# jina-ai/annlite

Measured on AMD Instinct MI355X. Metric: queries/sec, higher is better.
Workload: dtype f32; 1 GPU; 10000000 x 128-dim float32, PQ m=16 ks=256, euclidean, batch 1024, k=10, exhaustive ADC scan + exact top-k; rows_total=10000000, rows_per_gpu=10000000, batch=1024, k=10, parallelism=row-shard x1, codes_layout=skewed, n_ranks=1, streams=1, query_batches=4, prewarm_steps=64, seed_exchange=False, seed_peers_emulated=0

## Files before the change

### annlite_amd/csrc/scan_q8.hip

```cpp
#include "scan_lists.h"

#ifndef ANNLITE_Q8_EXP
#define ANNLITE_Q8_EXP 0
#endif

namespace annlite {

#ifndef ANNLITE_Q8_WDEPTH
#define ANNLITE_Q8_WDEPTH 16
#endif
#ifndef ANNLITE_Q8_STAGE_DEPTH
#define ANNLITE_Q8_STAGE_DEPTH 8
#endif
#ifndef ANNLITE_Q8_THW_MASK
#define ANNLITE_Q8_THW_MASK 1
#endif
#ifndef ANNLITE_Q8_ROWQ
#define ANNLITE_Q8_ROWQ 1
#endif
#ifndef ANNLITE_Q8_BUILD_UNROLL
#define ANNLITE_Q8_BUILD_UNROLL 2
#endif
#ifndef ANNLITE_Q8_DEPTH
#define ANNLITE_Q8_DEPTH 8
#endif
#ifndef ANNLITE_Q8_SPLIT_DEPTH
#define ANNLITE_Q8_SPLIT_DEPTH 4
#endif
#ifndef ANNLITE_Q8_SPLIT_H
#define ANNLITE_Q8_SPLIT_H 11
#endif
#ifndef ANNLITE_Q8_SPLIT_BIAS
#define ANNLITE_Q8_SPLIT_BIAS 1
#endif

#define ANNLITE_LDS __attribute__((address_space(3)))
template <class T>
__device__ __forceinline__ T ldsv(uint32_t ad) {
    return *(volatile ANNLITE_LDS T *)(uintptr_t)ad;
}
template <class T>
__device__ __forceinline__ void ldsv_st(uint32_t ad, T v) {
    *(volatile ANNLITE_LDS T *)(uintptr_t)ad = v;
}
__device__ __forceinline__ uint32_t lds_add_u32(uint32_t ad, uint32_t v) {
    return __hip_atomic_fetch_add((ANNLITE_LDS uint32_t *)(uintptr_t)ad, v, __ATOMIC_RELAXED, __HIP_MEMORY_SCOPE_WORKGROUP);
}
__device__ __forceinline__ uint32_t lds_base_addr() {
    return (uint32_t)(uintptr_t)(ANNLITE_LDS unsigned char *)g_smem;
}

typedef const ScanArgs __attribute__((address_space(4))) *q8_kernarg_ptr;
__device__ __forceinline__ q8_kernarg_ptr q8_kernarg() { return (q8_kernarg_ptr)__builtin_amdgcn_kernarg_segment_ptr(); }
struct Q8Build {
    const float *lut, *qlom, *qstep, *smax;
    const double *qlo;
    const unsigned long long *gkey;
    int32_t Ks, B, k, target;
    const unsigned long long *gseed0;
    const uint8_t *btab;
};

template <int M, int NW, int NQ>
__device__ __forceinline__ void q8_copy_table(const Q8Build &a, int tile, uint32_t tab_ad, int tid) {
    constexpr int NT = NW * 64;
    static_assert(M == 16 && NQ == 2, "the prebuilt image is the M = 16 kernel's (q8_entry16)");
    constexpr int n16 = kQ8Image16 / 16;
    const int n_g4 = ((a.B + 15) / 16) * 4;
    const u32x4 *src = (const u32x4 *)(a.btab + (int64_t)tile * (int64_t)kQ8Image16);
#pragma unroll 4
    for (int i = tid; i < n16; i += NT) {
        u32x4 v = src[i];
        const int half = i >= 4096 ? 1 : 0;
        const int g4 = tile * (4 * NQ) + (((i & 15) - half) & 1) * 4;
        if (g4 + 3 >= n_g4) {
            if (g4 + 0 >= n_g4) v.x = 0u;
            if (g4 + 1 >= n_g4) v.y = 0u;
            if (g4 + 2 >= n_g4) v.z = 0u;
            v.w = 0u;
        }
        *(ANNLITE_LDS u32x4 *)(uintptr_t)(tab_ad + 16u * (uint32_t)i) = v;
    }
}

template <int M, int NW, int NQ>
__device__ __forceinline__ void q8_build_table(const Q8Build &a, int tile, uint32_t tab_ad, uint32_t inv_ad, uint32_t clip_ad,
                                               int tid) {
    constexpr int RB = M * 16, NT = NW * 64, KHS = NT / M;
    static_assert(NT % M == 0 && KHS % NQ == 0, "build mapping");
    const int m = tid % M, kh0 = tid / M, h = kh0 % NQ;
    const int n_g4 = ((a.B + 15) / 16) * 4;
    float lo_r[16], inv_r[16], clip_r[16];
    const float *src[4];
#pragma unroll
    for (int i = 0; i < 4; ++i) {
        const int g4 = tile * (4 * NQ) + h * 4 + i;
        const bool ok = g4 < n_g4;
        src[i] = a.lut + ((int64_t)(ok ? g4 : 0) * a.Ks * M + m) * 4;
#pragma unroll
        for (int e = 0; e < 4; ++e) {
            lo_r[4 * i + e] = ok ? a.qlom[(int64_t)(g4 * 4 + e) * M + m] : 0.f;
            inv_r[4 * i + e] = ok ? ldsv<float>(inv_ad + 4u * (uint32_t)(h * 16 + 4 * i + e)) : 0.f;
            clip_r[4 * i + e] = ldsv<float>(clip_ad + 4u * (uint32_t)(h * 16 + 4 * i + e));
        }
    }
#pragma unroll ANNLITE_Q8_BUILD_UNROLL
    for (int kh = kh0; kh < a.Ks * NQ; kh += KHS) {
        const int k = kh / NQ;
        uint32_t w[4];
#pragma unroll
        for (int i = 0; i < 4; ++i) {
            const f32x4 v = *(const f32x4 *)(src[i] + (int64_t)k * M * 4);
            uint32_t pk = 0;
#pragma unroll
            for (int e = 0; e < 4; ++e) {
                float t = __builtin_fmaf(v[e] - lo_r[4 * i + e], inv_r[4 * i + e], -0.5f);
                t = __builtin_fminf(t, clip_r[4 * i + e]);
                pk = __builtin_amdgcn_cvt_pk_u8_f32(t, e, pk);
            }
            w[i] = pk;
        }
        uint32_t ad;
        if constexpr (Q8Cfg<M>::M32)
            ad = tab_ad + ((uint32_t)(m >> 4) << 16) + ((uint32_t)k << 8) + (uint32_t)(m & 15) * 16u;
        else if constexpr (M == 16 && NQ == 2) ad = tab_ad + q8_entry16((uint32_t)k, (uint32_t)m, (uint32_t)h);
        else ad = tab_ad + (uint32_t)((k * NQ + h) * RB + m * 16);
        *(ANNLITE_LDS u32x4 *)(uintptr_t)ad = (u32x4){w[0], w[1], w[2], w[3]};
    }
}

template <int NW>
__device__ __forceinline__ void q8_gather_table(const uint8_t *bq, int Ks, uint32_t tab_ad, uint32_t qmap_ad, int tid) {
    const int lane = tid & 63, wave = tid >> 6;
    const uint32_t w = (uint32_t)lane & 3u, g = ((uint32_t)lane >> 2) & 1u, u = ((uint32_t)lane >> 3) & 1u, c2 = (uint32_t)lane >> 4;
    int32_t qb[16];
#pragma unroll
    for (int j = 0; j < 16; ++j) {
        const int b = ldsv<int32_t>(qmap_ad + 4u * (g * 16u + (uint32_t)j));
        qb[j] = b < 0 ? -1 : b * (Ks * 16);
    }
    for (int kk = (int)(2u * c2 + u) + 8 * wave; kk < Ks; kk += 8 * NW) {
        uint32_t r[16];
#pragma unroll
        for (int j = 0; j < 16; ++j)
            r[j] = qb[j] < 0 ? 0u : *(const uint32_t *)(bq + (int64_t)qb[j] + (int64_t)(kk * 16) + (int64_t)(4u * w));
        u32x4 e[4];
#pragma unroll
        for (int v = 0; v < 4; ++v) {
            const uint32_t a = __builtin_amdgcn_perm(r[4 * v + 1], r[4 * v + 0], 0x05010400u);
            const uint32_t a2 = __builtin_amdgcn_perm(r[4 * v + 1], r[4 * v + 0], 0x07030602u);
            const uint32_t c = __builtin_amdgcn_perm(r[4 * v + 3], r[4 * v + 2], 0x05010400u);
            const uint32_t cc2 = __builtin_amdgcn_perm(r[4 * v + 3], r[4 * v + 2], 0x07030602u);
            e[0][v] = __builtin_amdgcn_perm(c, a, 0x05040100u);
            e[1][v] = __builtin_amdgcn_perm(c, a, 0x07060302u);
            e[2][v] = __builtin_amdgcn_perm(cc2, a2, 0x05040100u);
            e[3][v] = __builtin_amdgcn_perm(cc2, a2, 0x07060302u);
        }
#pragma unroll
        for (int t = 0; t < 4; ++t) {
            const uint32_t tt = (uint32_t)t ^ (2u * u);
            const u32x4 val = tt == 0u ? e[0] : tt == 1u ? e[1] : tt == 2u ? e[2] : e[3];
            *(ANNLITE_LDS u32x4 *)(uintptr_t)(tab_ad + q8_entry16((uint32_t)kk, 4u * w + tt, g)) = val;
        }
    }
}

template <int NW>
__device__ __forceinline__ void q8_build_table_wide(const Q8Build &a, int tile, uint32_t tab_ad, uint32_t inv_ad, uint32_t clip_ad,
                                                    int tid) {
    constexpr int M = 64, NT = NW * 64, KPT = NT / M;
    const int m = tid % M, kr = tid / M;
    const int n_g4 = ((a.B + 15) / 16) * 4;
    const uint32_t half_b = (uint32_t)(a.Ks + 1) * 256u;
    float lo_r[8], inv_r[8], clip_r[8];
    const float *src[2];
#pragma unroll
    for (int i = 0; i < 2; ++i) {
        const int g4 = tile * 2 + i;
        const bool ok = g4 < n_g4;
        src[i] = a.lut + ((int64_t)(ok ? g4 : 0) * a.Ks * M + m) * 4;
#pragma unroll
        for (int e = 0; e < 4; ++e) {
            lo_r[4 * i + e] = ok ? a.qlom[(int64_t)(g4 * 4 + e) * M + m] : 0.f;
            inv_r[4 * i + e] = ok ? ldsv<float>(inv_ad + 4u * (uint32_t)(4 * i + e)) : 0.f;
            clip_r[4 * i + e] = ldsv<float>(clip_ad + 4u * (uint32_t)(4 * i + e));
        }
// ... 1057 lines not shown
                    if (arrived == want) break;
                    if ((++idle & 15) == 8) {
                        import_bounds();
                        poll_guard();
                    }
                    __builtin_amdgcn_s_sleep(4);
                }
                q8_publish_global<QT, LK, TL>(fc, lds, lane, pend_o, pend_j);
                epoch_sync(final);
                if (final) break;
                if (ldsv<uint32_t>(lds.ctl)) {
                    if (has_ring && RE == 8u) {
                        const uint32_t tail_v = ldsv<uint32_t>(lds.tails() + 4u * (uint32_t)my_ring);
                        for (uint32_t i = (uint32_t)my_i; i < ((tail_v - head_v) & 0xffffu); i += 4u) {
                            const uint32_t ad = lds.ring + 8u * ((uint32_t)my_ring * kWaveRing + ((head_v + i) & (kWaveRing - 1)));
                            ldsv_st<unsigned long long>(ad, ldsv<unsigned long long>(ad) & ~(0xffffull << 40));
                        }
                    }
                }
                ++epoch;
                epoch_step = a.q8_epoch_mul * epoch_step + (a.q8_epoch_mul - 1);
            }
            if (a.guard && lane == 0) ldsv_st<uint32_t>(lds.seen, ldsv<uint32_t>(lds.seen) + n_seen);
            if (a.dbg && lane == 0 && !(a.dbg_skip & 8)) {
                atomicAdd(a.dbg + 2, (unsigned long long)n_kept);
                atomicAdd(a.dbg + 3, (unsigned long long)n_offered);
                atomicAdd(a.dbg + 4, t_busy);
                atomicAdd(a.dbg + 6, (unsigned long long)n_batches);
            }
        } else {
            constexpr int NF = WIDE ? 4 : 4 * NQ;
            int lane_pin = lane;
            asm volatile("" : "+v"(lane_pin));
            const int s = lane_pin % (WIDE ? 32 : M);
            const int rot_bytes = CB * s;
            const uint32_t bsh = (uint32_t)(rot_bytes & 3);
            bool abit[8];
#pragma unroll
            for (int i = 0; i < 8; ++i) abit[i] = (((rot_bytes >> 2) >> i) & 1) != 0;
            const unsigned long long rmask0 = __ballot(abit[0]), rmask1 = __ballot(abit[1]);
            typedef const ANNLITE_LDS u32x4 *lds_entry_ptr;
            typedef const ANNLITE_LDS u32x2 *lds_entry8_ptr;
            const uint32_t lds0 = lds.tab;
            constexpr bool P16 = M == 16 && NQ == 2 && CB == 1;
            uint32_t mbase[(WIDE || M8 || M32) ? 1 : M];
            if constexpr (!WIDE && !M8 && !M32) {
#pragma unroll
                for (int t = 0; t < M; ++t) mbase[t] = P16 ? q8_entry16(0u, (uint32_t)((s + t) % M), 0u) : lds0 + (uint32_t)(((s + t) % M) * EB);
                if constexpr (P16) {
                    if (lds0 != 0u) __builtin_trap();
                }
            }
            const uint32_t f16 = (M8 && NQ == 2) ? ((uint32_t)lane_pin >> 4) & 1u : 0u;
            uint32_t kx[2] = {0u, 0u}, ky[2] = {0u, 0u};
            if constexpr (M8) {
#pragma unroll
                for (int t = 0; t < 8; ++t) {
                    const uint32_t col = (uint32_t)(((s + t) % 8) * 16) + f16 * 128u;
                    kx[t / 4] |= col << (8 * (t % 4));
                    ky[t / 4] |= (col ^ 128u) << (8 * (t % 4));
                }
                if ((NQ == 2 && lds0 != 0u) || a.Ks > (C16 ? 1024 / NQ : 256)) __builtin_trap();
            }
            uint32_t mcol[(M8 && NQ == 1) ? M : 1];
            if constexpr (M8 && NQ == 1) {
#pragma unroll
                for (int t = 0; t < M; ++t) mcol[t] = lds0 + (uint32_t)(((s + t) % M) * EB);
            }
            uint32_t k32[M32 ? 16 : 1];
            if constexpr (M32) {
#pragma unroll
                for (int j = 0; j < 16; ++j) {
                    const uint32_t s0 = (uint32_t)((s + 2 * j) % 32), s1 = (uint32_t)((s + 2 * j + 1) % 32);
                    k32[j] = ((s0 & 15u) << 4) | ((s0 >> 4) << 8) | ((s1 & 15u) << 20) | ((s1 >> 4) << 24);
                }
                if (lds0 != 0u || a.Ks > 256) __builtin_trap();
            }
            const uint32_t lane_k = 0x00010000u | (uint32_t)((lane_pin & 31) * 8);
            if constexpr (WIDE) {
                if (lds0 != 0u || a.Ks != 256) __builtin_trap();
            }
            const uint32_t *codes32 = (const uint32_t *)a.codes;
            unsigned long long codes_v = (unsigned long long)(uintptr_t)a.codes, valid_v = (unsigned long long)(uintptr_t)a.valid;
            if constexpr (WIDE) asm volatile("" : "+v"(codes_v), "+v"(valid_v));
            const uint32_t n_rows = (uint32_t)a.N;
            const uint32_t n_blocks = item_blocks;
            const bool ilv = a.q8_ilv_log > 0;
            const uint32_t blk_log = ilv ? (uint32_t)a.q8_ilv_log : 26u, blk_msk = (1u << blk_log) - 1u;
            const uint32_t blk_per = ilv ? (uint32_t)a.n_slices << blk_log : 0u;
            const uint32_t blk_off = ilv ? ((uint32_t)slice << blk_log) << 6 : (uint32_t)slice_begin;
            const uint32_t s_end = ilv ? n_rows : (uint32_t)slice_end;
            auto blk_row = [&](uint32_t b) -> uint32_t { return blk_off + (((b >> blk_log) * blk_per + (b & blk_msk)) << 6); };
            auto draw = [&]() -> uint32_t {
                uint32_t v = 0;
                if (lane == 0) v = lds_add_u32(lds.blk_ctr(), 1u);
                return v;
            };
            uint32_t ccur[CW], cnext[CW];
            uint32_t addr[(WIDE || M8 || M32) ? 1 : M];
            auto load_row = [&](uint32_t row, uint32_t (&c)[CW]) {
                if constexpr (ANNLITE_Q8_EXP == 3) {
#pragma unroll
                    for (int i = 0; i < CW; ++i) c[i] = row * 0x9E3779B1u + (uint32_t)i * 0x85EBCA77u;
                    return;
                }
                if (row >= n_rows) row = n_rows - 1;
                typedef const uint32_t __attribute__((address_space(1))) *gptr_t;
                const gptr_t p = (WIDE ? (gptr_t)codes_v : (gptr_t)(uintptr_t)codes32) + (int64_t)row * CW;
                if constexpr (CW == 2) {
                    const u32x2 v = *(const u32x2 __attribute__((address_space(1))) *)p;
                    c[0] = v.x;
                    c[1] = v.y;
                } else {
#pragma unroll
                    for (int i = 0; i < CW / 4; ++i) {
                        const u32x4 v = *(const u32x4 __attribute__((address_space(1))) *)(p + 4 * i);
                        c[4 * i + 0] = v.x;
                        c[4 * i + 1] = v.y;
                        c[4 * i + 2] = v.z;
                        c[4 * i + 3] = v.w;
                    }
                }
            };
            auto make_addr = [&](const uint32_t (&cc)[CW]) {
                if constexpr (P16)
                    static_for<0, M>([&](auto T) {
                        constexpr int t = decltype(T)::value;
                        addr[t] = __builtin_amdgcn_perm(cc[t / 4], mbase[t], 0x0c020000u | ((4u + (uint32_t)(t % 4)) << 8));
                    });
                else if constexpr (!WIDE && !M8 && !M32)
                    static_for<0, CW>([&](auto W) {
                        constexpr int w = decltype(W)::value;
                        uint32_t o0, o1, o2, o3;
                        byte_shl4(cc[w], (uint32_t)ilog2_c(KSTRIDE), o0, o1, o2, o3);
                        addr[4 * w + 0] = mbase[4 * w + 0] + o0;
                        addr[4 * w + 1] = mbase[4 * w + 1] + o1;
                        addr[4 * w + 2] = mbase[4 * w + 2] + o2;
                        addr[4 * w + 3] = mbase[4 * w + 3] + o3;
                    });
            };
            auto load_thw = [&](uint32_t (&t)[NF]) {
                if constexpr (WIDE) {
                    const u32x4 v = *(volatile ANNLITE_LDS u32x4 *)(uintptr_t)lds.shq;
                    t[0] = v.x, t[1] = v.y, t[2] = v.z, t[3] = v.w;
                } else {
#pragma unroll
                    for (int h = 0; h < NQ; ++h) {
                        const u32x4 v = *(volatile ANNLITE_LDS u32x4 *)(uintptr_t)(lds.shq + 16u * ((uint32_t)h ^ f16));
                        t[4 * h + 0] = v.x, t[4 * h + 1] = v.y, t[4 * h + 2] = v.z, t[4 * h + 3] = v.w;
                    }
                }
            };
            constexpr bool BIAS = HS > 0 && ANNLITE_Q8_SPLIT_BIAS != 0;
            auto load_stepw = [&](uint32_t (&t)[NF]) {
                if constexpr (BIAS) {
#pragma unroll
                    for (int h = 0; h < 2; ++h) {
                        const u32x4 v = *(volatile ANNLITE_LDS u32x4 *)(uintptr_t)(lds.qmap + 16u * (uint32_t)h);
                        t[4 * h + 0] = v.x, t[4 * h + 1] = v.y, t[4 * h + 2] = v.z, t[4 * h + 3] = v.w;
                    }
                } else load_thw(t);
            };
            uint32_t thw[NF];
            load_stepw(thw);
            auto row_sums = [&](const uint32_t (&cc)[CW], uint32_t (&sums)[NF]) {
                if constexpr (WIDE) {
                    sums[0] = sums[1] = sums[2] = sums[3] = 0u;
                    constexpr int WDEPTH = ANNLITE_Q8_WDEPTH;
                    static_assert(WDEPTH % 2 == 0 && WDEPTH >= 2 && WDEPTH <= 64, "pairs");
                    u32x2 v[WDEPTH];
                    auto fetch = [&](u32x2 &dst, auto T) {
                        constexpr int t = decltype(T)::value;
                        constexpr int half = t / 32;
                        constexpr uint32_t sel = 0x0c000000u | ((half ? 0x02u : 0x0cu) << 16) | ((4u + (uint32_t)(t % 4)) << 8);
                        const uint32_t ad = __builtin_amdgcn_perm(cc[t / 4], lane_k, sel);
                        dst = *(lds_entry8_ptr)(uintptr_t)(ad + (uint32_t)((t % 32) * 8 + half * 0x100));
                    };
                    static_for<0, WDEPTH>([&](auto I) { fetch(v[decltype(I)::value], I); });
                    u32x2 bs = {0u, 0u};
                    static_for<0, 32>([&](auto P) {
                        constexpr int i = 2 * decltype(P)::value;
                        asm volatile("" ::: "memory");
                        if constexpr (i % 16 == 0) bs = v[i % WDEPTH] + v[(i + 1) % WDEPTH];
                        else bs += v[i % WDEPTH] + v[(i + 1) % WDEPTH];
                        if constexpr (i + WDEPTH < 64) {
                            fetch(v[i % WDEPTH], std::integral_constant<int, i + WDEPTH>{});
                            fetch(v[(i + 1) % WDEPTH], std::integral_constant<int, i + WDEPTH + 1>{});
                        }
                        if constexpr (i % 16 == 14) {
                            sums[0] += bs.x & 0x00ff00ffu;
                            sums[1] += __builtin_amdgcn_perm(0u, bs.x, 0x0c030c01u);
                            sums[2] += bs.y & 0x00ff00ffu;
                            sums[3] += __builtin_amdgcn_perm(0u, bs.y, 0x0c030c01u);
                        }
                    });
                } else if constexpr (M8) {
                    constexpr int DEPTH = ANNLITE_Q8_DEPTH, TOT = NQ * M;
                    u32x4 acc[NQ];
                    u32x4 v[DEPTH];
                    auto fetch = [&](u32x4 &dst, auto I) {
                        constexpr int i = decltype(I)::value, t = i % M, g = i / M;
                        constexpr uint32_t sel = C16 ? 0x0c000000u | ((uint32_t)(4 + 2 * (t % 2) + 1) << 16) | ((uint32_t)(4 + 2 * (t % 2)) << 8) | (uint32_t)(t % 4)
                                                     : 0x0c0c0000u | ((uint32_t)(4 + t % 4) << 8) | (uint32_t)(t % 4);
                        uint32_t ad;
                        if constexpr (NQ == 2) ad = __builtin_amdgcn_perm(cc[C16 ? t / 2 : t / 4], g ? ky[t / 4] : kx[t / 4], sel);
                        else ad = (((t % 2) ? cc[t / 2] >> 16 : cc[t / 2] & 0xffffu) << 7) + mcol[t];
                        dst = *(lds_entry_ptr)(uintptr_t)ad;
                    };
                    static_for<0, DEPTH>([&](auto I) { fetch(v[decltype(I)::value], I); });
                    static_for<0, TOT>([&](auto I) {
                        constexpr int i = decltype(I)::value;
                        asm volatile("" ::: "memory");
                        if constexpr (i % M == 0) acc[i / M] = v[i % DEPTH];
                        else acc[i / M] += v[i % DEPTH];
                        if constexpr (i + DEPTH < TOT) fetch(v[i % DEPTH], std::integral_constant<int, i + DEPTH>{});
                    });
#pragma unroll
                    for (int h = 0; h < NQ; ++h) sums[4 * h + 0] = acc[h].x, sums[4 * h + 1] = acc[h].y, sums[4 * h + 2] = acc[h].z, sums[4 * h + 3] = acc[h].w;
                } else if constexpr (M32) {
                    constexpr int DEPTH = ANNLITE_Q8_DEPTH;
                    u32x4 acc;
                    u32x4 v[DEPTH];
                    auto fetch = [&](u32x4 &dst, auto I) {
                        constexpr int t = decltype(I)::value, b = t % 2;
                        constexpr uint32_t sel = 0x0c000000u | ((uint32_t)(2 * b + 1) << 16) | ((uint32_t)(4 + t % 4) << 8) | (uint32_t)(2 * b);
                        const uint32_t ad = __builtin_amdgcn_perm(cc[t / 4], k32[t / 2], sel);
                        dst = *(lds_entry_ptr)(uintptr_t)ad;
                    };
                    static_for<0, DEPTH>([&](auto I) { fetch(v[decltype(I)::value], I); });
                    static_for<0, M>([&](auto I) {
                        constexpr int i = decltype(I)::value;
                        asm volatile("" ::: "memory");
                        if constexpr (i == 0) acc = v[0];
                        else acc += v[i % DEPTH];
                        if constexpr (i + DEPTH < M) fetch(v[i % DEPTH], std::integral_constant<int, i + DEPTH>{});
                    });
                    sums[0] = acc.x, sums[1] = acc.y, sums[2] = acc.z, sums[3] = acc.w;
                } else {
                    constexpr int DEPTH = ANNLITE_Q8_DEPTH, TOT = NQ * M;
                    constexpr int GOFF = P16 ? 16 : RB;
                    u32x4 acc[NQ];
                    u32x4 v[DEPTH];
                    auto fetch = [&](u32x4 &dst, uint32_t ad) {
                        if constexpr (ANNLITE_Q8_EXP == 2) asm volatile("" : "=v"(dst) : "v"(ad));
                        else dst = *(lds_entry_ptr)(uintptr_t)ad;
                    };
                    static_for<0, DEPTH>([&](auto I) {
                        constexpr int i = decltype(I)::value;
                        fetch(v[i], addr[i % M] + (uint32_t)((i / M) * GOFF));
                    });
                    static_for<0, TOT>([&](auto I) {
                        constexpr int i = decltype(I)::value;
                        asm volatile("" ::: "memory");
                        if constexpr (ANNLITE_Q8_EXP == 1) {
                            asm volatile("" ::"v"(v[i % DEPTH]));
                            if constexpr (i % M == 0) acc[i / M] = (u32x4){thw[4 * (i / M)], thw[4 * (i / M) + 1], thw[4 * (i / M) + 2], thw[4 * (i / M) + 3]};
                        } else {
                            if constexpr (i % M == 0) acc[i / M] = v[i % DEPTH];
                            else acc[i / M] += v[i % DEPTH];
                        }
                        if constexpr (i + DEPTH < TOT) {
                            constexpr int j = i + DEPTH;
                            fetch(v[i % DEPTH], addr[j % M] + (uint32_t)((j / M) * GOFF));
                        }
                    });
#pragma unroll
                    for (int h = 0; h < NQ; ++h) sums[4 * h + 0] = acc[h].x, sums[4 * h + 1] = acc[h].y, sums[4 * h + 2] = acc[h].z, sums[4 * h + 3] = acc[h].w;
                }
            };
            auto hits = [&](uint32_t th, uint32_t sm) -> uint32_t {
                if constexpr (WIDE) return (th - sm) & 0x80008000u;
                else return (th - (sm & 0x7f7f7f7fu)) & ~sm & 0x80808080u;
            };
            auto split_sums = [&](const uint32_t (&cc)[CW], auto T0c, auto T1c, auto DEPTHc, auto ONFLY, uint32_t sp, u32x4 (&acc)[2]) {
                constexpr int T0 = decltype(T0c)::value, TOT = 2 * (decltype(T1c)::value - T0);
                constexpr int DEPTH = decltype(DEPTHc)::value < TOT ? decltype(DEPTHc)::value : TOT;
                if constexpr (P16) {
                    if constexpr (decltype(ONFLY)::value) asm volatile("" : "+v"(sp));
                    u32x4 v[DEPTH];
                    uint32_t ad = 0;
                    auto fetch = [&](u32x4 &dst, auto I) {
                        constexpr int i = decltype(I)::value, t = T0 + i / 2;
                        if constexpr (i % 2 == 0) {
                            uint32_t mb;
                            if constexpr (decltype(ONFLY)::value) {
                                const uint32_t m = (sp + (uint32_t)t) & 15u;
                                mb = ((m & 1u) << 16) | (m << 4);
                            } else mb = mbase[t];
                            ad = __builtin_amdgcn_perm(cc[t / 4], mb, 0x0c020000u | ((4u + (uint32_t)(t % 4)) << 8));
                        }
                        dst = *(lds_entry_ptr)(uintptr_t)(ad + (uint32_t)((i % 2) * 16));
                    };
                    static_for<0, DEPTH>([&](auto I) { fetch(v[decltype(I)::value], I); });
                    static_for<0, TOT>([&](auto I) {
                        constexpr int i = decltype(I)::value;
                        asm volatile("" ::: "memory");
                        if constexpr (T0 == 0 && i < 2) acc[i] = v[i % DEPTH];
                        else acc[i % 2] += v[i % DEPTH];
                        if constexpr (decltype(ONFLY)::value) asm volatile("" : "+v"(acc[i % 2]));
                        if constexpr (i + DEPTH < TOT) fetch(v[i % DEPTH], std::integral_constant<int, i + DEPTH>{});
                    });
                }
            };
            auto split_pass = [&](const u32x4 (&acc)[2]) -> bool {
                uint32_t anyv = 0;
#pragma unroll
                for (int h = 0; h < 2; ++h)
#pragma unroll
                    for (int e = 0; e < 4; ++e) anyv |= (thw[4 * h + e] - (acc[h][e] & 0x7f7f7f7fu)) & ~acc[h][e];
                return (anyv & 0x80808080u) != 0u;
            };
            auto split_pass1 = [&](const u32x4 (&acc)[2]) -> bool {
                uint32_t allv = ~0u;
#pragma unroll
                for (int h = 0; h < 2; ++h)
#pragma unroll
                    for (int e = 0; e < 4; ++e) allv &= acc[h][e];
                return (~allv & 0x80808080u) != 0u;
            };
            const uint32_t sv_ad = lds.qmap + 128u + (uint32_t)wave * (uint32_t)(kSplitRing * 4);
            constexpr int HS1 = HS > 0 ? HS : 1;
            uint32_t sv_h = 0, sv_c = 0;
            uint32_t n_rows_a = 0, n_surv = 0, n_tail = 0, n_fb = 0;
            constexpr int PD = HS > 0 ? (ANNLITE_Q8_DEPTH < 2 * HS1 ? ANNLITE_Q8_DEPTH : 2 * HS1) : 1;
            u32x4 ring[PD];
            auto split_fetch = [&](u32x4 &dst, const uint32_t (&cc)[CW], uint32_t &ad, auto I) {
                constexpr int i = decltype(I)::value, t = i / 2;
                if constexpr (i % 2 == 0) ad = __builtin_amdgcn_perm(cc[t / 4], mbase[t], 0x0c020000u | ((4u + (uint32_t)(t % 4)) << 8));
                dst = *(lds_entry_ptr)(uintptr_t)(ad + (uint32_t)((i % 2) * 16));
            };
            auto split_prefix = [&](const auto &cc) {
                uint32_t ad = 0;
                static_for<0, PD>([&](auto I) { split_fetch(ring[decltype(I)::value], cc, ad, I); });
            };
            auto split_first = [&](auto &acc) {
                constexpr int TOT = 2 * HS1;
                u32x4 nr[PD];
                uint32_t ad = 0, an = 0;
                static_for<0, TOT>([&](auto I) {
                    constexpr int i = decltype(I)::value, j = i + PD;
                    if constexpr ((BIAS || j >= TOT) && i % 4 == 0 && i > 0) asm volatile("" : "+v"(acc[0]), "+v"(acc[1])::"memory");
                    else asm volatile("" ::: "memory");
                    if constexpr (i < 2) {
                        if constexpr (BIAS) acc[i] = ring[i % PD] + (u32x4){thw[4 * i], thw[4 * i + 1], thw[4 * i + 2], thw[4 * i + 3]};
                        else acc[i] = ring[i % PD];
                    } else acc[i % 2] += ring[i % PD];
                    if constexpr (j < TOT) split_fetch(ring[j % PD], ccur, ad, std::integral_constant<int, j>{});
                    else split_fetch(nr[j - TOT], cnext, an, std::integral_constant<int, j - TOT>{});
                });
#pragma unroll
                for (int i = 0; i < PD; ++i) ring[i] = nr[i];
            };
            auto split_head = [&](auto vmask, uint32_t row0, u32x4 (&acc)[2]) -> bool {
                split_first(acc);
                bool pass;
                if constexpr (BIAS) pass = split_pass1(acc);
                else pass = split_pass(acc);
                const unsigned long long alive = __ballot(pass) & vmask;
                const uint32_t n = (uint32_t)__popcll(alive);
                if (a.dbg) n_rows_a += (uint32_t)__popcll(vmask);
                if (n > (uint32_t)q8_split_fallback<HS1>()) return true;
                if (n) {
                    const uint32_t rank = __builtin_amdgcn_mbcnt_hi((uint32_t)(alive >> 32), __builtin_amdgcn_mbcnt_lo((uint32_t)alive, 0u));
                    if (__builtin_amdgcn_inverse_ballot_w64(alive))
                        ldsv_st<uint32_t>(sv_ad + 4u * ((sv_h + sv_c + rank) & (uint32_t)(kSplitRing - 1)), row0 + (uint32_t)lane);
                    sv_c += n;
                    n_surv += n;
                }
                return false;
            };
            auto split_finish = [&](auto vmask, u32x4 (&acc)[2]) -> unsigned long long {
                uint32_t sp = (uint32_t)s;
                asm volatile("" : "+v"(sp));
                split_sums(ccur, std::integral_constant<int, HS1>{}, std::integral_constant<int, 16>{}, std::integral_constant<int, ANNLITE_Q8_SPLIT_DEPTH>{}, std::true_type{}, sp, acc);
                ++n_fb;
                return __ballot(split_pass(acc)) & vmask;
            };
            uint32_t vcur = ~0u, vnext = ~0u;
            const uint32_t *valid = a.valid;
            auto load_valid = [&](uint32_t row) -> uint32_t {
                if (!valid) return ~0u;
                if (row >= n_rows) row = n_rows - 1;
                if constexpr (WIDE) return ((const uint32_t __attribute__((address_space(1))) *)valid_v)[row >> 5];
                else return valid[row >> 5];
            };
            uint32_t rs = 0;
            uint32_t n_slow = 0, n_push = 0;
            auto push_rows = [&](unsigned long long rem, uint32_t rid) {
                ++n_slow;
                const uint32_t n = (uint32_t)__popcll(rem);
                uint32_t tl = rs & 0xffffu, hd = rs >> 16;
                while (((tl + n - hd) & 0xffffu) > (uint32_t)kWaveRing) {
                    hd = ldsv<uint32_t>(lds.heads() + 4u * (uint32_t)wave) & 0xffffu;
                    if (((tl + n - hd) & 0xffffu) <= (uint32_t)kWaveRing) break;
                    __builtin_amdgcn_s_sleep(8);
                }
                const uint32_t rank = __builtin_amdgcn_mbcnt_hi((uint32_t)(rem >> 32), __builtin_amdgcn_mbcnt_lo((uint32_t)rem, 0u));
                if (__builtin_amdgcn_inverse_ballot_w64(rem))
                    ldsv_st<uint32_t>(lds.ring + RE * ((uint32_t)wave * kWaveRing + ((tl + rank) & (kWaveRing - 1))),
                                      rid);
                tl = (tl + n) & 0xffffu;
                if (lane == 0) ldsv_st<uint32_t>(lds.tails() + 4u * (uint32_t)wave, tl);
                rs = tl | (hd << 16);
                n_push += n;
            };
            auto split_tail = [&](auto nb) {
                const bool on = (uint32_t)lane < nb;
                const uint32_t rid = ldsv<uint32_t>(sv_ad + 4u * ((sv_h + (on ? (uint32_t)lane : 0u)) & (uint32_t)(kSplitRing - 1)));
                uint32_t cb[CW];
                load_row(rid, cb);
                uint32_t sp = (uint32_t)s;
                asm volatile("" : "+v"(sp));
                const uint32_t r = (sp - rid) & 15u;
                {
                    const bool q1 = (r & 4u) != 0u, q2 = (r & 8u) != 0u;
                    uint32_t d[CW];
#pragma unroll
                    for (int i = 0; i < CW; ++i) d[i] = q1 ? cb[(i + 1) % CW] : cb[i];
#pragma unroll
                    for (int i = 0; i < CW; ++i) cb[i] = q2 ? d[(i + 2) % CW] : d[i];
#pragma unroll
                    for (int i = 0; i < CW; ++i) d[i] = __builtin_amdgcn_alignbyte(cb[(i + 1) % CW], cb[i], r & 3u);
#pragma unroll
                    for (int i = 0; i < CW; ++i) cb[i] = d[i];
                }
                u32x4 acc[2];
                split_sums(cb, std::integral_constant<int, 0>{}, std::integral_constant<int, 16>{}, std::integral_constant<int, ANNLITE_Q8_SPLIT_DEPTH>{}, std::true_type{}, sp, acc);
                const unsigned long long rem = __ballot(on && split_pass(acc));
                if (rem && !(a.dbg_skip & 4)) push_rows(rem, rid);
                ++n_tail;
            };
            uint32_t b_cur = (uint32_t)__builtin_amdgcn_readfirstlane((int)draw());
            uint32_t pend = draw();
            load_row(blk_row(b_cur) + lane, cnext);
            vnext = load_valid(blk_row(b_cur) + lane);
            uint32_t b_nxt = (uint32_t)__builtin_amdgcn_readfirstlane((int)pend);
            uint32_t it_no = 0;
            const uint32_t thw_mask = (uint32_t)a.q8_thw_mask;
            unsigned long long t_wait = 0;
            for (int epoch_step = a.q8_epoch0;; epoch_step = a.q8_epoch_mul * epoch_step + (a.q8_epoch_mul - 1)) {
                const bool final = TL || epoch_step >= n_steps - 1;
                const uint32_t end_blk = final ? n_blocks : (uint32_t)NS * (uint32_t)(epoch_step + 1);
                if constexpr (HS > 0) {
                    asm volatile("" ::"v"(cnext[0]), "v"(cnext[1]), "v"(cnext[2]), "v"(cnext[3]), "v"(vnext));
                    split_prefix(cnext);
                }
                for (; b_cur < end_blk; ++it_no) {
                    const uint32_t row0 = blk_row(b_cur);
                    pend = draw();
                    constexpr bool ROT4 = !SKEWED && !WIDE && CW == 4;
                    uint32_t rot1[ROT4 ? CW : 1];
                    if constexpr (ROT4) {
#pragma unroll
                        for (int i = 0; i < CW; ++i)
                            asm("v_cndmask_b32 %0, %1, %2, %3" : "=v"(rot1[i]) : "v"(cnext[i]), "v"(cnext[(i + 1) % CW]), "s"(rmask0));
                    } else {
#pragma unroll
                        for (int i = 0; i < CW; ++i) ccur[i] = cnext[i];
                    }
                    vcur = vnext;
                    {
                        const uint32_t row1 = blk_row(b_nxt) + lane;
                        load_row(row1, cnext);
                        vnext = load_valid(row1);
                    }
                    if constexpr (!SKEWED) {
                        if constexpr (WIDE) skew64_encode(ccur, lane & 31);
                        else if constexpr (ROT4) {
                            uint32_t n[CW];
#pragma unroll
                            for (int i = 0; i < CW; ++i)
                                asm("v_cndmask_b32 %0, %1, %2, %3" : "=v"(n[i]) : "v"(rot1[i]), "v"(rot1[(i + 2) % CW]), "s"(rmask1));
#pragma unroll
                            for (int i = 0; i < CW; ++i) ccur[i] = __builtin_amdgcn_alignbyte(n[(i + 1) % CW], n[i], bsh);
                        } else rotate_row<CW>(ccur, abit, bsh);
                    }
                    unsigned long long vmask = ~0ull;
                    if (s_end - row0 < 64u) vmask = (1ull << (s_end - row0)) - 1ull;
                    if (valid) vmask &= __ballot((vcur >> (lane & 31)) & 1u);
                    uint32_t sums[NF];
                    unsigned long long rem;
                    if constexpr (HS > 0) {
                        u32x4 acc[2];
                        const bool fb = split_head(vmask, row0, acc);
                        if (fb || sv_c >= 64u) {
                            if constexpr (BIAS) {
                                if (fb) {
#pragma unroll
                                    for (int h = 0; h < 2; ++h)
#pragma unroll
                                        for (int e = 0; e < 4; ++e) acc[h][e] -= thw[4 * h + e];
                                }
                                asm volatile("" ::: "memory");
                                load_thw(thw);
                            }
                            if (fb) {
                                rem = split_finish(vmask, acc);
                                if (rem && !(a.dbg_skip & 4)) push_rows(rem, row0 + (uint32_t)lane);
                            }
                            if (sv_c >= 64u) {
                                split_tail(64u);
                                sv_h ^= 64u;
                                sv_c -= 64u;
                            }
                            asm volatile("" ::: "memory");
                            split_prefix(cnext);
                            if constexpr (BIAS) load_stepw(thw);
                        }
                    } else {
                        make_addr(ccur);
                        row_sums(ccur, sums);
                        uint32_t anyv = 0;
                        if constexpr (WIDE) {
#pragma unroll
                            for (int w = 0; w < NF; ++w) anyv |= thw[w] - sums[w];
                            anyv &= 0x80008000u;
                        } else {
#pragma unroll
                            for (int w = 0; w < NF; ++w) anyv |= (thw[w] - (sums[w] & 0x7f7f7f7fu)) & ~sums[w];
                            anyv &= 0x80808080u;
                        }
                        rem = __ballot(anyv != 0) & vmask;
                    }
                    if constexpr (ROWQ) {
                        if constexpr (HS == 0)
                            if (rem && !(a.dbg_skip & 4)) push_rows(rem, row0 + (uint32_t)lane);
                    } else
                    if (rem && !(a.dbg_skip & 4)) {
                        ++n_slow;
                        uint32_t ts[NF];
#pragma unroll
                        for (int i = 0; i < NF; ++i) ts[i] = (uint32_t)__builtin_amdgcn_readfirstlane((int)thw[i]);
                        uint32_t e_lo = 0, e_hi = 0;
                        int n = 0;
                        for (;;) {
                            if (n > 32 || (n > 0 && !rem)) {
                                uint32_t tl = rs & 0xffffu, hd = rs >> 16;
                                while (((tl + (uint32_t)n - hd) & 0xffffu) > (uint32_t)kWaveRing) {
                                    hd = ldsv<uint32_t>(lds.heads() + 4u * (uint32_t)wave) & 0xffffu;
                                    if (((tl + (uint32_t)n - hd) & 0xffffu) <= (uint32_t)kWaveRing) break;
                                    __builtin_amdgcn_s_sleep(8);
                                }
                                if (lane < n)
                                    ldsv_st<unsigned long long>(lds.ring + 8u * ((uint32_t)wave * kWaveRing + ((tl + (uint32_t)lane) & (kWaveRing - 1))),
                                                                ((unsigned long long)e_hi << 32) | e_lo);
                                tl = (tl + (uint32_t)n) & 0xffffu;
                                if (lane == 0) ldsv_st<uint32_t>(lds.tails() + 4u * (uint32_t)wave, tl);
                                rs = tl | (hd << 16);
                                n_push += (uint32_t)n;
                                n = 0;
                            }
                            if (!rem) break;
                            const int L = __builtin_ctzll(rem);
                            rem &= rem - 1ull;
                            const uint32_t rid = row0 + (uint32_t)L;
                            const uint32_t fL = M8 ? ((uint32_t)L >> 4) & 1u : 0u;
                            if constexpr (ANNLITE_Q8_EXP == 5) {
                                if (lane == n) {
                                    e_hi = (uint32_t)L & 31u;
                                    e_lo = rid;
                                }
                                ++n;
                                continue;
                            }
                            static_for<0, NF>([&](auto I) {
                                constexpr int i = decltype(I)::value;
                                const uint32_t ss = (uint32_t)__builtin_amdgcn_readlane((int)sums[i], L);
                                if constexpr (M8 && NQ == 2) ts[i] = (uint32_t)__builtin_amdgcn_readlane((int)thw[i], L);
                                uint32_t bits = hits(ts[i], ss);
                                while (bits) {
                                    uint32_t sv, slot;
                                    if constexpr (WIDE) {
                                        const uint32_t hf = (uint32_t)__builtin_ctz(bits) >> 4;
                                        sv = (ss >> (16u * hf)) & 0xffffu;
                                        slot = (uint32_t)((i & 2) << 1) | (hf << 1) | (uint32_t)(i & 1);
                                    } else {
                                        const uint32_t by = (uint32_t)__builtin_ctz(bits) >> 3;
                                        sv = (ss >> (8u * by)) & 0xffu;
                                        slot = (uint32_t)(4 * i) + by;
                                        if constexpr (M8 && NQ == 2) slot ^= fL << 4;
                                    }
                                    bits &= bits - 1u;
                                    if (lane == n) {
                                        e_hi = (sv << 8) | slot;
                                        e_lo = rid;
                                    }
                                    ++n;
                                }
                            });
                        }
                    }
                    if ((it_no & thw_mask) == thw_mask) {
                        asm volatile("" ::: "memory");
                        load_stepw(thw);
                    }
                    b_cur = b_nxt;
                    b_nxt = (uint32_t)__builtin_amdgcn_readfirstlane((int)pend);
                }
                if constexpr (HS > 0) {
                    if (sv_c) {
                        if constexpr (BIAS) load_thw(thw);
                        split_tail(sv_c);
                    }
                    sv_h = sv_c = 0u;
                }
                if (lane == 0) lds_add_u32(lds.arrived(), 1u);
                const unsigned long long tw = a.dbg ? __builtin_readcyclecounter() : 0ull;
                if (final) stamp(2);
                epoch_sync(final);
                if (a.dbg) t_wait += __builtin_readcyclecounter() - tw;
                if (final) stamp(3);
                if (final) break;
                load_stepw(thw);
            }
            if (a.dbg && lane == 0 && !(a.dbg_skip & 8)) {
                atomicAdd(a.dbg + 0, (unsigned long long)n_slow);
                atomicAdd(a.dbg + 1, (unsigned long long)n_push);
                if (wave == 0) atomicAdd(a.dbg + 7, t_wait);
                if constexpr (HS > 0) {
                    atomicAdd(a.dbg + kDbgSplit + 0, (unsigned long long)n_rows_a);
                    atomicAdd(a.dbg + kDbgSplit + 1, (unsigned long long)n_surv);
                    atomicAdd(a.dbg + kDbgSplit + 2, (unsigned long long)n_tail);
                    atomicAdd(a.dbg + kDbgSplit + 3, (unsigned long long)n_fb);
                }
            }
        }

        q8_finish_item<M, NW, NQ, LK, TL>(ka, tile, slice);
        if (a.dbg && tid == 0) {
            const unsigned long long t_end = wall_clock64();
            const unsigned long long t_item = ldsv<unsigned long long>(stamp_ad), t_built = ldsv<unsigned long long>(stamp_ad + 8),
                                     t_scanned = ldsv<unsigned long long>(stamp_ad + 16), t_synced = ldsv<unsigned long long>(stamp_ad + 24);
            atomicMax(a.dbg + 8, (1ull << 62) - t_item);
            atomicMax(a.dbg + 9, t_end);
            atomicAdd(a.dbg + 10, t_item);
            atomicAdd(a.dbg + 11, t_built - t_item);
            atomicAdd(a.dbg + 12, t_scanned - t_built);
            atomicAdd(a.dbg + 13, t_synced - t_scanned);
            atomicAdd(a.dbg + 14, t_end - t_synced);
            const unsigned long long rec = atomicAdd(a.dbg + 15, 1ull);
            if (rec < 4096ull) {
                unsigned long long *r = a.dbg + 16 + rec * 8;
                r[0] = (unsigned long long)tile;
                r[1] = (unsigned long long)slice;
                r[2] = t_item;
                r[3] = t_built;
                r[4] = t_scanned;
                r[5] = t_synced;
                r[6] = t_end;
                r[7] = (unsigned long long)blockIdx.x;
            }
        }
    }
    if constexpr (!M8) {
        if (blockIdx.x == 0 && tid == 0) {
            unsigned long long *clk = ka->clk;
            if (clk) clk[2] = __builtin_readcyclecounter(), clk[3] = wall_clock64();
        }
    }
    if (a.guard) {
        __syncthreads();
        if (tid == 0) {
            __hip_atomic_fetch_add((unsigned long long *)(a.guard + 2), (unsigned long long)ldsv<uint32_t>(lds.seen), __ATOMIC_RELAXED,
                                   __HIP_MEMORY_SCOPE_AGENT);
            const unsigned int old = __hip_atomic_fetch_add(a.guard + 1, 1u, __ATOMIC_ACQ_REL, __HIP_MEMORY_SCOPE_AGENT);
            if (old + 1u == gridDim.x - 1u && a.host_stats) {
                const unsigned long long seen =
                    __hip_atomic_load((unsigned long long *)(a.guard + 2), __ATOMIC_RELAXED, __HIP_MEMORY_SCOPE_AGENT) + 1ull;
                const unsigned int gave_up = __hip_atomic_load(a.guard, __ATOMIC_RELAXED, __HIP_MEMORY_SCOPE_AGENT) == 0u ? 1u : 0u;
                __hip_atomic_store(a.host_stats + 1, gave_up, __ATOMIC_RELAXED, __HIP_MEMORY_SCOPE_SYSTEM);
                __hip_atomic_store(a.host_stats + 2, (unsigned int)seen, __ATOMIC_RELAXED, __HIP_MEMORY_SCOPE_SYSTEM);
                __hip_atomic_store(a.host_stats + 3, (unsigned int)(seen >> 32), __ATOMIC_RELAXED, __HIP_MEMORY_SCOPE_SYSTEM);
                __hip_atomic_store(a.host_stats + 4, (unsigned int)a.B, __ATOMIC_RELAXED, __HIP_MEMORY_SCOPE_SYSTEM);
                __hip_atomic_store(a.host_stats + 5, (unsigned int)a.N, __ATOMIC_RELAXED, __HIP_MEMORY_SCOPE_SYSTEM);
                __hip_atomic_store(a.host_stats + 0, a.stats_seq, __ATOMIC_RELEASE, __HIP_MEMORY_SCOPE_SYSTEM);
            }
        }
    }
}
// ... 57 lines not shown
```

Before: 969,500 queries/s.

## Unroll split scan loop by two with ping-pong code buffers and pinned addresses

Moves the split-path block loop into a dedicated split_step lambda and unrolls it twice, swapping the current and next code buffers in place of copying cnext into ccur every iteration. It pins LDS base addresses, lane offsets and the debug flag in registers through inline asm constraints, and adds a direct clamped 128-bit global load for code blocks and survivor rows. The aim is to remove register copies and address recomputation in the hot ADC scan loop, at the cost of larger code size and more register pressure.

```diff
diff --git a/annlite_amd/csrc/scan_q8.hip b/annlite_amd/csrc/scan_q8.hip
--- a/annlite_amd/csrc/scan_q8.hip
+++ b/annlite_amd/csrc/scan_q8.hip
@@ -32,6 +32,9 @@
 #endif
 #ifndef ANNLITE_Q8_SPLIT_BIAS
 #define ANNLITE_Q8_SPLIT_BIAS 1
+#endif
+#ifndef ANNLITE_Q8_SPLIT_UNROLL
+#define ANNLITE_Q8_SPLIT_UNROLL 1
 #endif
 
 #define ANNLITE_LDS __attribute__((address_space(3)))
@@ -1395,11 +1398,13 @@
                 }
             };
             constexpr bool BIAS = HS > 0 && ANNLITE_Q8_SPLIT_BIAS != 0;
+            uint32_t shq_v = lds.shq;
+            if constexpr (HS > 0) asm volatile("" : "+v"(shq_v));
             auto load_stepw = [&](uint32_t (&t)[NF]) {
                 if constexpr (BIAS) {
 #pragma unroll
                     for (int h = 0; h < 2; ++h) {
-                        const u32x4 v = *(volatile ANNLITE_LDS u32x4 *)(uintptr_t)(lds.qmap + 16u * (uint32_t)h);
+                        const u32x4 v = *(volatile ANNLITE_LDS u32x4 *)(uintptr_t)(shq_v + (lds.qmap - lds.shq) + 16u * (uint32_t)h);
                         t[4 * h + 0] = v.x, t[4 * h + 1] = v.y, t[4 * h + 2] = v.z, t[4 * h + 3] = v.w;
                     }
                 } else load_thw(t);
@@ -1562,9 +1567,12 @@
                 return (~allv & 0x80808080u) != 0u;
             };
             const uint32_t sv_ad = lds.qmap + 128u + (uint32_t)wave * (uint32_t)(kSplitRing * 4);
+            const uint32_t sv_wave = (uint32_t)wave * (uint32_t)(kSplitRing * 4);
             constexpr int HS1 = HS > 0 ? HS : 1;
             uint32_t sv_h = 0, sv_c = 0;
             uint32_t n_rows_a = 0, n_surv = 0, n_tail = 0, n_fb = 0;
+            uint32_t dbg_on = (uint32_t)(uintptr_t)a.dbg | (uint32_t)((unsigned long long)(uintptr_t)a.dbg >> 32);
+            if constexpr (HS > 0) asm volatile("" : "+s"(dbg_on));
             constexpr int PD = HS > 0 ? (ANNLITE_Q8_DEPTH < 2 * HS1 ? ANNLITE_Q8_DEPTH : 2 * HS1) : 1;
             u32x4 ring[PD];
             auto split_fetch = [&](u32x4 &dst, const uint32_t (&cc)[CW], uint32_t &ad, auto I) {
@@ -1576,7 +1584,7 @@
                 uint32_t ad = 0;
                 static_for<0, PD>([&](auto I) { split_fetch(ring[decltype(I)::value], cc, ad, I); });
             };
-            auto split_first = [&](auto &acc) {
+            auto split_first = [&](auto &acc, const auto &cc, const auto &cn) {
                 constexpr int TOT = 2 * HS1;
                 u32x4 nr[PD];
                 uint32_t ad = 0, an = 0;
@@ -1588,34 +1596,40 @@
                         if constexpr (BIAS) acc[i] = ring[i % PD] + (u32x4){thw[4 * i], thw[4 * i + 1], thw[4 * i + 2], thw[4 * i + 3]};
                         else acc[i] = ring[i % PD];
                     } else acc[i % 2] += ring[i % PD];
-                    if constexpr (j < TOT) split_fetch(ring[j % PD], ccur, ad, std::integral_constant<int, j>{});
-                    else split_fetch(nr[j - TOT], cnext, an, std::integral_constant<int, j - TOT>{});
+                    if constexpr (j < TOT) split_fetch(ring[j % PD], cc, ad, std::integral_constant<int, j>{});
+                    else split_fetch(nr[j - TOT], cn, an, std::integral_constant<int, j - TOT>{});
                 });
 #pragma unroll
                 for (int i = 0; i < PD; ++i) ring[i] = nr[i];
             };
-            auto split_head = [&](auto vmask, uint32_t row0, u32x4 (&acc)[2]) -> bool {
-                split_first(acc);
+            auto split_head = [&](auto vmask, uint32_t row0, u32x4 (&acc)[2], const auto &cc, const auto &cn) -> bool {
+                split_first(acc, cc, cn);
                 bool pass;
                 if constexpr (BIAS) pass = split_pass1(acc);
                 else pass = split_pass(acc);
                 const unsigned long long alive = __ballot(pass) & vmask;
-                const uint32_t n = (uint32_t)__popcll(alive);
-                if (a.dbg) n_rows_a += (uint32_t)__popcll(vmask);
+                uint32_t n = (uint32_t)__popcll(alive);
+                asm("" : "+s"(n));
+                uint32_t dbg_now = dbg_on;
+                asm volatile("" : "+s"(dbg_now));
+                if (dbg_now != 0u) {
+                    asm volatile("");
+                    n_rows_a += (uint32_t)__popcll(vmask);
+                }
                 if (n > (uint32_t)q8_split_fallback<HS1>()) return true;
                 if (n) {
                     const uint32_t rank = __builtin_amdgcn_mbcnt_hi((uint32_t)(alive >> 32), __builtin_amdgcn_mbcnt_lo((uint32_t)alive, 0u));
                     if (__builtin_amdgcn_inverse_ballot_w64(alive))
-                        ldsv_st<uint32_t>(sv_ad + 4u * ((sv_h + sv_c + rank) & (uint32_t)(kSplitRing - 1)), row0 + (uint32_t)lane);
+                        ldsv_st<uint32_t>(shq_v + sv_wave + 4u * ((sv_h + sv_c + rank) & (uint32_t)(kSplitRing - 1)) + (lds.qmap + 128u - lds.shq), row0 + (uint32_t)lane);
                     sv_c += n;
                     n_surv += n;
                 }
                 return false;
             };
-            auto split_finish = [&](auto vmask, u32x4 (&acc)[2]) -> unsigned long long {
+            auto split_finish = [&](auto vmask, u32x4 (&acc)[2], const auto &cc) -> unsigned long long {
                 uint32_t sp = (uint32_t)s;
                 asm volatile("" : "+v"(sp));
-                split_sums(ccur, std::integral_constant<int, HS1>{}, std::integral_constant<int, 16>{}, std::integral_constant<int, ANNLITE_Q8_SPLIT_DEPTH>{}, std::true_type{}, sp, acc);
+                split_sums(cc, std::integral_constant<int, HS1>{}, std::integral_constant<int, 16>{}, std::integral_constant<int, ANNLITE_Q8_SPLIT_DEPTH>{}, std::true_type{}, sp, acc);
                 ++n_fb;
                 return __ballot(split_pass(acc)) & vmask;
             };
@@ -1626,6 +1640,25 @@
                 if (row >= n_rows) row = n_rows - 1;
                 if constexpr (WIDE) return ((const uint32_t __attribute__((address_space(1))) *)valid_v)[row >> 5];
                 else return valid[row >> 5];
+            };
+            uint32_t lane16 = (uint32_t)lane_pin * 16u, lane_w4 = ((uint32_t)lane_pin >> 5) * 4u, lane_bit = 1u << (lane_pin & 31);
+            if constexpr (HS > 0) asm volatile("" : "+v"(lane16), "+v"(lane_w4), "+v"(lane_bit));
+            auto load_block = [&](uint32_t r, uint32_t (&c)[CW], uint32_t &v) {
+                if constexpr (CW != 4 || ANNLITE_Q8_EXP == 3) {
+                    load_row(r + (uint32_t)lane, c);
+                    v = load_valid(r + (uint32_t)lane);
+                } else {
+                    const uint32_t last = n_rows - 1u;
+                    const uint32_t rb = r < last ? r : last, room = last - rb;
+                    const uint32_t lim16 = room < 64u ? room * 16u : 63u * 16u, limw = (room >> 5) != 0u ? 4u : 0u;
+                    unsigned long long cb = (unsigned long long)(uintptr_t)codes32 + (unsigned long long)rb * 16u;
+                    unsigned long long vb = (unsigned long long)(uintptr_t)valid + (unsigned long long)(rb >> 5) * 4u;
+                    asm("" : "+s"(cb), "+s"(vb));
+                    const uint32_t o16 = lane16 < lim16 ? lane16 : lim16, ow4 = lane_w4 < limw ? lane_w4 : limw;
+                    const u32x4 w = *(const u32x4 __attribute__((address_space(1))) *)(cb + o16);
+                    if (valid) v = *(const uint32_t __attribute__((address_space(1))) *)(vb + ow4);
+                    c[0] = w.x, c[1] = w.y, c[2] = w.z, c[3] = w.w;
+                }
             };
             uint32_t rs = 0;
             uint32_t n_slow = 0, n_push = 0;
@@ -1651,7 +1684,12 @@
                 const bool on = (uint32_t)lane < nb;
                 const uint32_t rid = ldsv<uint32_t>(sv_ad + 4u * ((sv_h + (on ? (uint32_t)lane : 0u)) & (uint32_t)(kSplitRing - 1)));
                 uint32_t cb[CW];
-                load_row(rid, cb);
+                if constexpr (CW != 4 || ANNLITE_Q8_EXP == 3) load_row(rid, cb);
+                else {
+                    const uint32_t rr = rid < s_end - 1u ? rid : s_end - 1u;
+                    const u32x4 w = *(const u32x4 __attribute__((address_space(1))) *)((const uint32_t __attribute__((address_space(1))) *)(uintptr_t)codes32 + (int64_t)rr * CW);
+                    cb[0] = w.x, cb[1] = w.y, cb[2] = w.z, cb[3] = w.w;
+                }
                 uint32_t sp = (uint32_t)s;
                 asm volatile("" : "+v"(sp));
                 const uint32_t r = (sp - rid) & 15u;
@@ -1688,6 +1726,67 @@
                     asm volatile("" ::"v"(cnext[0]), "v"(cnext[1]), "v"(cnext[2]), "v"(cnext[3]), "v"(vnext));
                     split_prefix(cnext);
                 }
+                auto split_step = [&](auto &cc, auto &cn, uint32_t &vc, uint32_t &vn) {
+                    const uint32_t row0 = blk_row(b_cur);
+                    asm volatile("" : "=v"(pend));
+                    if (lane == 0) pend = lds_add_u32(shq_v + (lds.blk_ctr() - lds.shq), lane_bit);
+                    load_block(blk_row(b_nxt), cn, vn);
+                    unsigned long long vmask = ~0ull;
+                    if (s_end - row0 < 64u) vmask = (1ull << (s_end - row0)) - 1ull;
+                    if (valid) vmask &= __ballot((vc & lane_bit) != 0u);
+                    u32x4 acc[2];
+                    const bool fb = split_head(vmask, row0, acc, cc, cn);
+                    if (fb || sv_c >= 64u) {
+                        if constexpr (BIAS) {
+                            if (fb) {
+#pragma unroll
+                                for (int h = 0; h < 2; ++h)
+#pragma unroll
+                                    for (int e = 0; e < 4; ++e) acc[h][e] -= thw[4 * h + e];
+                            }
+                            asm volatile("" ::: "memory");
+                            load_thw(thw);
+                        }
+                        if (fb) {
+                            const unsigned long long rem = split_finish(vmask, acc, cc);
+                            if (rem && !(a.dbg_skip & 4)) push_rows(rem, row0 + (uint32_t)lane);
+                        }
+                        if (sv_c >= 64u) {
+                            split_tail(64u);
+                            sv_h ^= 64u;
+                            sv_c -= 64u;
+                        }
+                        asm volatile("" ::: "memory");
+                        split_prefix(cn);
+                        if constexpr (BIAS) load_stepw(thw);
+                    }
+                    if ((it_no & thw_mask) == thw_mask) {
+                        asm volatile("" ::: "memory");
+                        load_stepw(thw);
+                    }
+                    b_cur = b_nxt;
+                    b_nxt = (uint32_t)__builtin_amdgcn_readfirstlane((int)pend);
+                    ++it_no;
+                };
+                if constexpr (HS > 0 && ANNLITE_Q8_SPLIT_UNROLL != 0) {
+                    while (b_cur < end_blk) {
+                        split_step(cnext, ccur, vnext, vcur);
+                        if (b_cur >= end_blk) {
+#pragma unroll
+                            for (int i = 0; i < CW; ++i) cnext[i] = ccur[i];
+                            vnext = vcur;
+                            break;
+                        }
+                        split_step(ccur, cnext, vcur, vnext);
+                    }
+                } else if constexpr (HS > 0) {
+                    while (b_cur < end_blk) {
+#pragma unroll
+                        for (int i = 0; i < CW; ++i) ccur[i] = cnext[i];
+                        vcur = vnext;
+                        split_step(ccur, cnext, vcur, vnext);
+                    }
+                } else
                 for (; b_cur < end_blk; ++it_no) {
                     const uint32_t row0 = blk_row(b_cur);
                     pend = draw();
@@ -1723,34 +1822,7 @@
                     if (valid) vmask &= __ballot((vcur >> (lane & 31)) & 1u);
                     uint32_t sums[NF];
                     unsigned long long rem;
-                    if constexpr (HS > 0) {
-                        u32x4 acc[2];
-                        const bool fb = split_head(vmask, row0, acc);
-                        if (fb || sv_c >= 64u) {
-                            if constexpr (BIAS) {
-                                if (fb) {
-#pragma unroll
-                                    for (int h = 0; h < 2; ++h)
-#pragma unroll
-                                        for (int e = 0; e < 4; ++e) acc[h][e] -= thw[4 * h + e];
-                                }
-                                asm volatile("" ::: "memory");
-                                load_thw(thw);
-                            }
-                            if (fb) {
-                                rem = split_finish(vmask, acc);
-                                if (rem && !(a.dbg_skip & 4)) push_rows(rem, row0 + (uint32_t)lane);
-                            }
-                            if (sv_c >= 64u) {
-                                split_tail(64u);
-                                sv_h ^= 64u;
-                                sv_c -= 64u;
-                            }
-                            asm volatile("" ::: "memory");
-                            split_prefix(cnext);
-                            if constexpr (BIAS) load_stepw(thw);
-                        }
-                    } else {
+                    {
                         make_addr(ccur);
                         row_sums(ccur, sums);
                         uint32_t anyv = 0;
@@ -1766,8 +1838,7 @@
                         rem = __ballot(anyv != 0) & vmask;
                     }
                     if constexpr (ROWQ) {
-                        if constexpr (HS == 0)
-                            if (rem && !(a.dbg_skip & 4)) push_rows(rem, row0 + (uint32_t)lane);
+                        if (rem && !(a.dbg_skip & 4)) push_rows(rem, row0 + (uint32_t)lane);
                     } else
                     if (rem && !(a.dbg_skip & 4)) {
                         ++n_slow;
```

Result: faster. 1.008 million queries/s, median of 6 (+3.9%).
